# XinMing0411/AC-VAE

Measured on AMD Instinct MI355X. Metric: train-step captions/s (and audio-sec/s) at B=32, 1/2/4/8 MI355X, higher is better.
Workload: dtype f32

## Files before the change

acvae_amd/csrc/conv_wino.hip:

```cpp
#include "mfma_tile.h"
#include "../../include/acvae_hip.h"
#include "conv.h"
#include "prof.h"
#include <type_traits>

namespace {
using namespace mfma;

constexpr int WN_THREADS = 256;
constexpr int WN_TILES = 32;
constexpr int WN_TN = 64;
constexpr int WN_SC = 66, WN_SR = 2 * WN_SC, WN_SQ = 276;
constexpr int WN_BCHUNK = 16 * 2 * 64;
constexpr int WN_MAXC = 2048;
#ifndef WN_PRIO_EDGE
#define WN_PRIO_EDGE 3
#endif
#ifndef WN_PF_DIST
#define WN_PF_DIST 64
#endif

constexpr int WN_RAWBUF = 4 * WN_SQ;
constexpr int WN_EX_F4 = 6 * 512;
constexpr int WN_LDS_F4 = WN_EX_F4 + 64;
static_assert(2 * WN_RAWBUF <= WN_LDS_F4 && 2 * WN_RAWBUF + 2 * WN_MAXC / 4 >= WN_LDS_F4, "exchange + sums overlay the window buffers (+ scale / shift)");

__device__ __forceinline__ void wino_tile(int row, int tw_shift, int& tyl, int& tx) {
  const int cell = (int)((0x1c0c081804141000ULL >> (8 * (row >> 2))) & 0xff) + (row & 3);
  if (tw_shift >= 4) {
    tyl = cell >> tw_shift;
    tx = cell & ((1 << tw_shift) - 1);
  } else {
    const int g = cell >> 4, l16 = cell & 15;
    tx = l16 & ((1 << tw_shift) - 1);
    tyl = g + 2 * (l16 >> tw_shift);
  }
}
__host__ __device__ __forceinline__ int wino_row_pitch(int tw_shift) {
  return tw_shift == 3 ? 12 : tw_shift == 2 ? 6 : (1 << tw_shift) + 1;
}

struct WinoParams {
  const float* X;
  const float* scale;
  const float* shift;
  const float* U;
  float* Y;
  float* partials;
  const float* rY;
  const float* rscale;
  const float* rshift;
  const float* rmean;
  const float* rinvstd;
  int N, H, W, C, Cout;
  int tw_shift;
  int R;
  int bpc;
  int w_shift;
  unsigned bpc_magic;
  int nn_shift;
  int bn_group;
};
__device__ __forceinline__ void wino_tile_of(const WinoParams& p, int t, int nm, int nn, int& bm, int& bn) {
  if (p.bn_group) {
    const int G = p.bn_group, per = nm * G;
    int grp = (int)__fdividef((float)t, (float)per);
    int rem = t - grp * per;
    if (rem < 0) { --grp; rem += per; } else if (rem >= per) { ++grp; rem -= per; }
    bm = rem >> (G >> 1);
    bn = grp * G + (rem & (G - 1));
  } else if (p.nn_shift >= 0) { bn = t & (nn - 1); bm = t >> p.nn_shift; }
  else { bn = t % nn; bm = t / nn; }
}
__device__ __forceinline__ int wino_xcd_tile(const WinoParams& p, int nm, int nn, int& bm, int& bn) {
  const int total = nm * nn;
  const int b = blockIdx.x + blockIdx.y * nm;
  const int q = total >> 3, r = total & 7;
  const int xcd = b & 7, idx = b >> 3;
  const int t = xcd * q + (xcd < r ? xcd : r) + idx;
  wino_tile_of(p, t, nm, nn, bm, bn);
  return t;
}

typedef float f32x2 __attribute__((ext_vector_type(2)));
#define WN_PK_SUB(d, a, b) "v_pk_add_f32 " d ", " a ", " b " neg_lo:[0,1] neg_hi:[0,1]\n\t"
#define WN_PK_ADD(d, a, b) "v_pk_add_f32 " d ", " a ", " b "\n\t"
__device__ __forceinline__ float4 f4sub(float4 a, float4 b) {
  f32x2 lo, hi;
  asm(WN_PK_SUB("%0", "%2", "%4") WN_PK_SUB("%1", "%3", "%5")
      : "=&v"(lo), "=&v"(hi) : "v"(f32x2{a.x, a.y}), "v"(f32x2{a.z, a.w}), "v"(f32x2{b.x, b.y}), "v"(f32x2{b.z, b.w}));
  return make_float4(lo[0], lo[1], hi[0], hi[1]);
}
__device__ __forceinline__ float4 f4add(float4 a, float4 b) {
  f32x2 lo, hi;
  asm(WN_PK_ADD("%0", "%2", "%4") WN_PK_ADD("%1", "%3", "%5")
      : "=&v"(lo), "=&v"(hi) : "v"(f32x2{a.x, a.y}), "v"(f32x2{a.z, a.w}), "v"(f32x2{b.x, b.y}), "v"(f32x2{b.z, b.w}));
  return make_float4(lo[0], lo[1], hi[0], hi[1]);
}
__device__ __forceinline__ void wino_htrans(const float4 (&t)[4], float4 (&v)[4]) {
  f32x2 o[8];
  asm(WN_PK_SUB("%0", "%8", "%12") WN_PK_SUB("%1", "%9", "%13")
      WN_PK_ADD("%2", "%10", "%12") WN_PK_ADD("%3", "%11", "%13")
      WN_PK_SUB("%4", "%12", "%10") WN_PK_SUB("%5", "%13", "%11")
      WN_PK_SUB("%6", "%10", "%14") WN_PK_SUB("%7", "%11", "%15")
      "s_nop 1"
      : "=&v"(o[0]), "=&v"(o[1]), "=&v"(o[2]), "=&v"(o[3]), "=&v"(o[4]), "=&v"(o[5]), "=&v"(o[6]), "=&v"(o[7])
      : "v"(f32x2{t[0].x, t[0].y}), "v"(f32x2{t[0].z, t[0].w}), "v"(f32x2{t[1].x, t[1].y}), "v"(f32x2{t[1].z, t[1].w}),
        "v"(f32x2{t[2].x, t[2].y}), "v"(f32x2{t[2].z, t[2].w}), "v"(f32x2{t[3].x, t[3].y}), "v"(f32x2{t[3].z, t[3].w}));
#pragma unroll
  for (int k = 0; k < 4; ++k) v[k] = make_float4(o[2 * k][0], o[2 * k][1], o[2 * k + 1][0], o[2 * k + 1][1]);
}
__device__ __forceinline__ void pk_sub_ip(float4& a, const float4& b) {
  f32x2 lo{a.x, a.y}, hi{a.z, a.w};
  asm(WN_PK_SUB("%0", "%0", "%2") WN_PK_SUB("%1", "%1", "%3") : "+v"(lo), "+v"(hi) : "v"(f32x2{b.x, b.y}), "v"(f32x2{b.z, b.w}));
  a = make_float4(lo[0], lo[1], hi[0], hi[1]);
}
__device__ __forceinline__ void pk_add_ip(float4& a, const float4& b) {
  f32x2 lo{a.x, a.y}, hi{a.z, a.w};
  asm(WN_PK_ADD("%0", "%0", "%2") WN_PK_ADD("%1", "%1", "%3") : "+v"(lo), "+v"(hi) : "v"(f32x2{b.x, b.y}), "v"(f32x2{b.z, b.w}));
  a = make_float4(lo[0], lo[1], hi[0], hi[1]);
}
__device__ __forceinline__ void wino_htrans_ip(float4 (&t)[4], float4 (&v)[4]) {
  f32x2 a0{t[0].x, t[0].y}, a1{t[0].z, t[0].w}, c0{t[2].x, t[2].y}, c1{t[2].z, t[2].w}, e0{t[3].x, t[3].y}, e1{t[3].z, t[3].w};
  f32x2 n0, n1;
  asm(WN_PK_SUB("%0", "%0", "%2") WN_PK_SUB("%1", "%1", "%3")
      WN_PK_ADD("%6", "%8", "%2") WN_PK_ADD("%7", "%9", "%3")
      WN_PK_SUB("%2", "%2", "%8") WN_PK_SUB("%3", "%3", "%9")
      WN_PK_SUB("%4", "%8", "%4") WN_PK_SUB("%5", "%9", "%5")
      "s_nop 1"
      : "+v"(a0), "+v"(a1), "+v"(c0), "+v"(c1), "+v"(e0), "+v"(e1), "=&v"(n0), "=&v"(n1)
      : "v"(f32x2{t[1].x, t[1].y}), "v"(f32x2{t[1].z, t[1].w}));
  v[0] = make_float4(a0[0], a0[1], a1[0], a1[1]);
  v[1] = make_float4(n0[0], n0[1], n1[0], n1[1]);
  v[2] = make_float4(c0[0], c0[1], c1[0], c1[1]);
  v[3] = make_float4(e0[0], e0[1], e1[0], e1[1]);
}
__device__ __forceinline__ void mfma4_first(f32x16& c, float4 a, float4 b) {
  const f32x16 z = {0.f, 0.f, 0.f, 0.f, 0.f, 0.f, 0.f, 0.f, 0.f, 0.f, 0.f, 0.f, 0.f, 0.f, 0.f, 0.f};
  c = __builtin_amdgcn_mfma_f32_32x32x2f32(a.x, b.x, z, 0, 0, 0);
  c = __builtin_amdgcn_mfma_f32_32x32x2f32(a.y, b.y, c, 0, 0, 0);
  c = __builtin_amdgcn_mfma_f32_32x32x2f32(a.z, b.z, c, 0, 0, 0);
  c = __builtin_amdgcn_mfma_f32_32x32x2f32(a.w, b.w, c, 0, 0, 0);
}
__device__ __forceinline__ void mfma4(f32x16& c, float4 a, float4 b) {
  c = __builtin_amdgcn_mfma_f32_32x32x2f32(a.x, b.x, c, 0, 0, 0);
  c = __builtin_amdgcn_mfma_f32_32x32x2f32(a.y, b.y, c, 0, 0, 0);
  c = __builtin_amdgcn_mfma_f32_32x32x2f32(a.z, b.z, c, 0, 0, 0);
  c = __builtin_amdgcn_mfma_f32_32x32x2f32(a.w, b.w, c, 0, 0, 0);
}

template <int XI, int MODE>
__device__ __forceinline__ void wino_epilogue(const WinoParams& p, const f32x16 (&acc)[8], float2* ex, float* red, int li, int h,
                                              int lane, int n, int ty0, int bm, int bn) {
  constexpr int ROW = XI >> 1, NH = XI & 1;
  constexpr int SET_OTHER = XI == 0 ? 0 : XI == 1 ? 1 : XI == 2 ? 4 : 5;
  constexpr int SET_OWN = XI == 1 ? 2 : XI == 2 ? 3 : -1;
  constexpr int SET_A = XI == 0 ? 1 : XI == 1 ? 0 : XI == 2 ? 1 : 2, SET_B = XI == 0 ? 3 : XI == 1 ? 4 : XI == 2 ? 5 : 4;
  constexpr bool STATS = MODE != 0;
  const int tid = XI * 64 + lane;
  const int H = p.H, W = p.W, Cout = p.Cout;
  const int cout = bn * WN_TN + NH * 32 + li;
  int yk[4], voff[4];
#pragma unroll
  for (int k = 0; k < 4; ++k) {
    int tyl, tx;
    wino_tile(8 * k + 4 * h, p.tw_shift, tyl, tx);
    yk[k] = 2 * (ty0 + tyl) + ROW;
    voff[k] = ((yk[k] * W + 2 * tx) * Cout + cout) * 4;
  }
  int dyj[4], soff[4];
#pragma unroll
  for (int j = 0; j < 4; ++j) {
    dyj[j] = p.tw_shift == 1 ? 4 * (j >> 1) : 0;
    const int dx = p.tw_shift == 1 ? 2 * (j & 1) : 2 * j;
    soff[j] = (dyj[j] * W + dx) * Cout * 4;
  }
  const int pix = Cout * 4;
  float2 yv[MODE == 2 ? 16 : 1];
  float rsc = 0.f, rsh = 0.f, rmu = 0.f, ris = 0.f;
  if (MODE == 2) {
    const __amdgpu_buffer_rsrc_t rrs = __builtin_amdgcn_make_buffer_rsrc(const_cast<float*>(p.rY) + (long)n * H * W * Cout, 0, H * W * Cout * 4, 0x00020000);
#pragma unroll
    for (int r = 0; r < 16; ++r) {
      yv[r].x = __uint_as_float(__builtin_amdgcn_raw_buffer_load_b32(rrs, voff[r >> 2], soff[r & 3], 0));
      yv[r].y = __uint_as_float(__builtin_amdgcn_raw_buffer_load_b32(rrs, voff[r >> 2], soff[r & 3] + pix, 0));
    }
    rsc = p.rscale[cout]; rsh = p.rshift[cout]; rmu = p.rmean[cout]; ris = p.rinvstd[cout];
  }
  float2 keep[16];
#pragma unroll
  for (int r = 0; r < 16; ++r) {
#pragma unroll
    for (int nh = 0; nh < 2; ++nh) {
      const float m0 = acc[0 + nh][r], m1 = acc[2 + nh][r], m2 = acc[4 + nh][r], m3 = acc[6 + nh][r];
      const float2 f = make_float2(m0 + m1 + m2, m1 - m2 - m3);
      if (nh == NH) {
        keep[r] = f;
        if (SET_OWN >= 0) ex[(SET_OWN * 16 + r) * 64 + lane] = f;
      } else {
        ex[(SET_OTHER * 16 + r) * 64 + lane] = f;
      }
    }
  }
  __syncthreads();
  const __amdgpu_buffer_rsrc_t yrs = __builtin_amdgcn_make_buffer_rsrc(p.Y + (long)n * H * W * Cout, 0, H * W * Cout * 4, 0x00020000);
  float s = 0.f, qq = 0.f;
#pragma unroll
  for (int r = 0; r < 16; ++r) {
    const int k = r >> 2, j = r & 3;
    const float2 a = ex[(SET_A * 16 + r) * 64 + lane], b = ex[(SET_B * 16 + r) * 64 + lane];
    const float o0 = ROW ? a.x - (b.x + keep[r].x) : (keep[r].x + a.x) + b.x, o1 = ROW ? a.y - (b.y + keep[r].y) : (keep[r].y + a.y) + b.y;
    __builtin_amdgcn_raw_buffer_store_b32(__float_as_uint(o0), yrs, voff[k], soff[j], 0);
    __builtin_amdgcn_raw_buffer_store_b32(__float_as_uint(o1), yrs, voff[k], soff[j] + pix, 0);
    if (MODE == 1) {
      const bool ok = yk[k] + dyj[j] < H;
      const float a0 = ok ? o0 : 0.f, a1 = ok ? o1 : 0.f;
      s += a0 + a1;
      qq += a0 * a0 + a1 * a1;
    }
    if (MODE == 2) {
      const bool ok = yk[k] + dyj[j] < H;
      const float g0 = (ok && yv[r].x * rsc + rsh > 0.f) ? o0 : 0.f, g1 = (ok && yv[r].y * rsc + rsh > 0.f) ? o1 : 0.f;
      s += g0; s += g1;
      qq += g0 * ((yv[r].x - rmu) * ris); qq += g1 * ((yv[r].y - rmu) * ris);
    }
  }
  if (STATS && p.partials) {
    s += __shfl_xor(s, 32, 64);
    qq += __shfl_xor(qq, 32, 64);
    if (h == 0) {
      red[(ROW * 2 + 0) * 64 + NH * 32 + li] = s;
      red[(ROW * 2 + 1) * 64 + NH * 32 + li] = qq;
    }
    __syncthreads();
    if (tid < WN_TN) {
      const float ts = red[(0 * 2 + 0) * 64 + tid] + red[(1 * 2 + 0) * 64 + tid], tq = red[(0 * 2 + 1) * 64 + tid] + red[(1 * 2 + 1) * 64 + tid];
      float* out = p.partials + (long)bm * 2 * p.Cout + bn * WN_TN + tid;
      out[0] = ts;
      out[p.Cout] = tq;
    }
  }
}

template <int XI, bool ACT, int STATS>
__device__ __forceinline__ void conv_wino_body(const WinoParams& p, float4* raw0, float4* raw1, float4* scsh) {
  __builtin_amdgcn_s_setprio(WN_PRIO_EDGE);
  const int tid = threadIdx.x, lane = tid & 63;
  const int li = lane & 31, h = lane >> 5;
  int bm, bn;
  const int tpos = wino_xcd_tile(p, gridDim.x, gridDim.y, bm, bn);
  const int RW = wino_row_pitch(p.tw_shift), R = p.R;
  const int n = p.bpc == 1 ? bm : (int)__umulhi((unsigned)bm, p.bpc_magic), ty0 = (bm - n * p.bpc) * R;
  const int H = p.H, W = p.W, C = p.C;

  const int nitems = ((2 * R + 2) << p.w_shift) * 4;
  const int q = tid & 3;
  for (int i = tid; i < (2 * R + 2) * 8; i += WN_THREADS) {
    const int ry = i >> 3, side = (i >> 2) & 1, qi = i & 3;
    const int rx = side ? W + 1 : 0;
    const int slot = qi * WN_SQ + (ry & 1) * WN_SR + (rx & 1) * WN_SC + (ry >> 1) * RW + (rx >> 1);
    raw0[slot] = make_float4(0.f, 0.f, 0.f, 0.f);
    raw1[slot] = make_float4(0.f, 0.f, 0.f, 0.f);
  }
  unsigned goff[4];
  int loff[4];
#pragma unroll
  for (int j = 0; j < 4; ++j) {
    const int e = tid + WN_THREADS * j;
    const bool lv = e < nitems;
    const int px = e >> 2;
    const int ry = px >> p.w_shift, x = px & (W - 1), rx = x + 1;
    const int y = 2 * ty0 - 1 + ry;
    const bool ok = lv && y >= 0 && y < H;
    goff[j] = ok ? (unsigned)((((long)(n * H + y) * W + x) * C) + q * 4) : 0u;
    const int slot = q * WN_SQ + (ry & 1) * WN_SR + (rx & 1) * WN_SC + (ry >> 1) * RW + (rx >> 1);
    if (lv && !ok) {
      raw0[slot] = make_float4(0.f, 0.f, 0.f, 0.f);
      raw1[slot] = make_float4(0.f, 0.f, 0.f, 0.f);
    }
    loff[j] = ok ? slot : WN_RAWBUF - 1 - (tid & 7);
  }
  float4 pv[4];
  auto issue_raw = [&](int st) {
#pragma unroll
    for (int j = 0; j < 4; ++j) pv[j] = *reinterpret_cast<const float4*>(p.X + goff[j] + st * 16);
  };
  auto stage_scsh = [&]() {
    if (ACT) {
      for (int i = tid; i < (C >> 2); i += WN_THREADS) {
        scsh[i] = *reinterpret_cast<const float4*>(p.scale + 4 * i);
        scsh[(C >> 2) + i] = *reinterpret_cast<const float4*>(p.shift + 4 * i);
      }
      __syncthreads();
    }
  };
  float4 sc = make_float4(1.f, 1.f, 1.f, 1.f), sh = make_float4(0.f, 0.f, 0.f, 0.f);
  auto read_scsh = [&](int st) {
    if (ACT) {
      sc = scsh[st * 4 + q];
      sh = scsh[(C >> 2) + st * 4 + q];
    }
  };
  auto put_raw_part = [&](float4* raw, int j0) {
#pragma unroll
    for (int j = j0; j < j0 + 2; ++j) {
      float4 v = pv[j];
      if (ACT) {
        v.x = fmaxf(v.x * sc.x + sh.x, 0.f); v.y = fmaxf(v.y * sc.y + sh.y, 0.f);
        v.z = fmaxf(v.z * sc.z + sh.z, 0.f); v.w = fmaxf(v.w * sc.w + sh.w, 0.f);
      }
      raw[loff[j]] = v;
    }
  };
  auto put_raw = [&](float4* raw) { put_raw_part(raw, 0); put_raw_part(raw, 2); };
  const int nchunk = C >> 3;
  const __amdgpu_buffer_rsrc_t urs = __builtin_amdgcn_make_buffer_rsrc(
      const_cast<float*>(p.U + ((long)bn * nchunk) * (WN_BCHUNK * 4)), 0, 0x7fffffff, 0x00020000);
  int tyl_a, tx_a;
  wino_tile(li, p.tw_shift, tyl_a, tx_a);
  const int abase = tyl_a * RW + tx_a;
  constexpr int RA = XI == 0 ? 0 : XI == 2 ? 2 : 1, RB = XI == 0 ? 2 : XI == 1 ? 2 : XI == 2 ? 1 : 3;
  const int rowa = (RA & 1) * WN_SR + (RA >> 1) * RW + abase, rowb = (RB & 1) * WN_SR + (RB >> 1) * RW + abase;
  const int bvoff = (h * 64 + li) * 16;
  auto load_b = [&](int c, int g) {
    typedef unsigned wn_v4u __attribute__((ext_vector_type(4)));
    const wn_v4u v = __builtin_amdgcn_raw_buffer_load_b128(urs, bvoff, c * (WN_BCHUNK * 16) + (XI * 4 + (g >> 1)) * 2048 + (g & 1) * 512, 0);
    return make_float4(__uint_as_float(v.x), __uint_as_float(v.y), __uint_as_float(v.z), __uint_as_float(v.w));
  };

  f32x16 acc[8];

  const int nstage = C >> 4;
  const float4* const aq0 = raw0 + h * WN_SQ;
  const float4* const aq1 = raw1 + h * WN_SQ;
  float4 va[4], vb[4], B[4];
  auto read_row = [&](const float4* rq, int row, float4 (&d)[4]) {
#pragma unroll
    for (int j = 0; j < 4; ++j) d[j] = rq[row + (j & 1) * WN_SC + (j >> 1)];
  };
  auto vertical = [&](float4 (&da)[4], float4 (&db)[4]) {
#pragma unroll
    for (int j = 0; j < 4; ++j) {
      if (XI == 1) pk_add_ip(da[j], db[j]); else pk_sub_ip(da[j], db[j]);
    }
  };

#pragma unroll
  for (int g = 0; g < 4; ++g) B[g] = load_b(0, g);
  issue_raw(0);
  stage_scsh();
  read_scsh(0);
  put_raw(raw0);
  issue_raw(nstage > 1 ? 1 : 0);
  __syncthreads();
  {
    float4 da[4], db[4];
    read_row(aq0, rowa, da);
    read_row(aq0, rowb, db);
    vertical(da, db);
    wino_htrans_ip(da, va);
  }
#define WN_SB() __builtin_amdgcn_sched_barrier(0)
  auto step = [&](int c, auto kk, auto first) {
    constexpr int K = decltype(kk)::value;
    constexpr bool FIRST = decltype(first)::value;
    auto mm = [&](f32x16& a_, float4 x_, float4 y_) { if (FIRST) mfma4_first(a_, x_, y_); else mfma4(a_, x_, y_); };
    constexpr int sub = K & 1, sp = K >> 1;
    float4 (&vc)[4] = sub ? vb : va;
    float4 (&vn)[4] = sub ? va : vb;
    const int st = c >> 1;
    float4* const rnxt = sp ? raw0 : raw1;
    const float4* const nq = sub ? (sp ? aq0 : aq1) : (sp ? aq1 : aq0) + 2 * WN_SQ;
    const int cn = c + 1 < nchunk ? c + 1 : c;
    float4 da[4], db[4];
    const int st1 = st + 1 < nstage ? st + 1 : nstage - 1, st2 = st + 2 < nstage ? st + 2 : nstage - 1;
    if (sub == 0) read_scsh(st1);
    WN_SB();
    mm(acc[0], vc[0], B[0]);
    WN_SB();
    B[0] = load_b(c, 4);
    if (sub == 0) put_raw_part(rnxt, 0);
    WN_SB();
    mm(acc[1], vc[0], B[1]);
    WN_SB();
    B[1] = load_b(c, 5);
    if (sub == 0) put_raw_part(rnxt, 2);
    WN_SB();
    mm(acc[2], vc[1], B[2]);
    WN_SB();
    B[2] = load_b(c, 6);
    if (sub == 0) issue_raw(st2);
    WN_SB();
    mm(acc[3], vc[1], B[3]);
    WN_SB();
    B[3] = load_b(c, 7);
    read_row(nq, rowa, da);
    WN_SB();
    mm(acc[4], vc[2], B[0]);
    WN_SB();
    B[0] = load_b(cn, 0);
    read_row(nq, rowb, db);
    WN_SB();
    mm(acc[5], vc[2], B[1]);
    WN_SB();
    B[1] = load_b(cn, 1);
    WN_SB();
    mm(acc[6], vc[3], B[2]);
    WN_SB();
    B[2] = load_b(cn, 2);
    vertical(da, db);
    WN_SB();
    mm(acc[7], vc[3], B[3]);
    WN_SB();
    B[3] = load_b(cn, 3);
    wino_htrans_ip(da, vn);
    WN_SB();
    if (sub == 0) __syncthreads();
  };
#undef WN_SB
  using std::integral_constant;
  using std::false_type;
  __builtin_amdgcn_s_setprio(0);
  step(0, integral_constant<int, 0>(), std::true_type());
  step(1, integral_constant<int, 1>(), false_type());
  if (2 < nchunk) {
    step(2, integral_constant<int, 2>(), false_type());
    step(3, integral_constant<int, 3>(), false_type());
  }
  for (int c = 4; c < nchunk; c += 4) {
    step(c, integral_constant<int, 0>(), false_type());
    step(c + 1, integral_constant<int, 1>(), false_type());
    if (c + 2 < nchunk) {
      step(c + 2, integral_constant<int, 2>(), false_type());
      step(c + 3, integral_constant<int, 3>(), false_type());
    }
  }
  __builtin_amdgcn_s_setprio(WN_PRIO_EDGE);
  __syncthreads();
  const int lane_e = (int)__builtin_amdgcn_mbcnt_hi(~0u, __builtin_amdgcn_mbcnt_lo(~0u, 0u));
  const int li_e = lane_e & 31, h_e = lane_e >> 5;
  const int tid_e = XI * 64 + lane_e;

  float pfv = 0.f;
  if (!ACT) {
    const int nn_ = (int)gridDim.y;
    const int t2 = tpos + WN_PF_DIST * ((int)gridDim.x * nn_ >= 8 * WN_PF_DIST ? 1 : 0);
    int bm2 = bm, bn2 = bn;
    if (t2 < (int)gridDim.x * nn_) wino_tile_of(p, t2, (int)gridDim.x, nn_, bm2, bn2);
    const int n2 = p.bpc == 1 ? bm2 : (int)__umulhi((unsigned)bm2, p.bpc_magic), ty2 = (bm2 - n2 * p.bpc) * R;
    const int ry = tid_e >> p.w_shift, x = tid_e & (W - 1);
    const int y = 2 * ty2 - 1 + ry;
    if (bm2 < (int)gridDim.x && bm2 != bm && ry < 2 * R + 2 && y >= 0 && y < H)
      pfv = p.X[((long)(n2 * H + y) * W + x) * C];
  }

  float2* exb = reinterpret_cast<float2*>(raw0);
  wino_epilogue<XI, STATS>(p, acc, exb, reinterpret_cast<float*>(raw0 + WN_EX_F4),
                           li_e, h_e, lane_e, n, ty0, bm, bn);
  if (!ACT) asm volatile("" :: "v"(pfv));
}

template <bool ACT, int STATS>
__device__ __forceinline__ void conv_wino_entry(const WinoParams& p, float4* raw, float4* scsh) {
  switch (threadIdx.x >> 6) {
    case 0: conv_wino_body<0, ACT, STATS>(p, raw, raw + WN_RAWBUF, scsh); break;
    case 1: conv_wino_body<1, ACT, STATS>(p, raw, raw + WN_RAWBUF, scsh); break;
    case 2: conv_wino_body<2, ACT, STATS>(p, raw, raw + WN_RAWBUF, scsh); break;
    default: conv_wino_body<3, ACT, STATS>(p, raw, raw + WN_RAWBUF, scsh); break;
  }
}
__global__ __launch_bounds__(WN_THREADS, 2) void conv_wino_kernel(WinoParams p) {
  __shared__ float4 raw[WN_LDS_F4];
  conv_wino_entry<false, 0>(p, raw, nullptr);
}
__global__ __launch_bounds__(WN_THREADS, 2) void conv_wino_bnred_kernel(WinoParams p) {
  __shared__ float4 raw[WN_LDS_F4];
  conv_wino_entry<false, 2>(p, raw, nullptr);
}
__global__ __launch_bounds__(WN_THREADS, 2) void conv_wino_stats_kernel(WinoParams p) {
  __shared__ float4 raw[WN_LDS_F4];
  conv_wino_entry<false, 1>(p, raw, nullptr);
}
__global__ __launch_bounds__(WN_THREADS, 2) void conv_wino_act_kernel(WinoParams p) {
  __shared__ float4 raw[2 * WN_RAWBUF + 2 * WN_MAXC / 4];
  conv_wino_entry<true, 1>(p, raw, raw + 2 * WN_RAWBUF);
}

__device__ __forceinline__ void wino_weights_item(const float* __restrict__ Wt, float4* __restrict__ U, int Cout, int Cin, int dgrad,
                                                  long idx) {
  const int K = dgrad ? Cout : Cin, NO = dgrad ? Cin : Cout;
  {
    const int out = (int)(idx % NO), kq = (int)(idx / NO);
    float u[16][4];
#pragma unroll
    for (int jj = 0; jj < 4; ++jj) {
      const int in = kq * 4 + jj;
      double g[3][3];
#pragma unroll
      for (int a = 0; a < 3; ++a)
#pragma unroll
        for (int b = 0; b < 3; ++b)
          g[a][b] = dgrad ? (double)Wt[((long)in * Cin + out) * 9 + (2 - a) * 3 + (2 - b)]
                          : (double)Wt[((long)out * Cin + in) * 9 + a * 3 + b];
      double t[4][3];
#pragma unroll
      for (int b = 0; b < 3; ++b) {
        t[0][b] = g[0][b];
        t[1][b] = 0.5 * (g[0][b] + g[1][b] + g[2][b]);
        t[2][b] = 0.5 * (g[0][b] - g[1][b] + g[2][b]);
        t[3][b] = g[2][b];
      }
#pragma unroll
      for (int xi = 0; xi < 4; ++xi) {
        u[xi * 4 + 0][jj] = (float)t[xi][0];
        u[xi * 4 + 1][jj] = (float)(0.5 * (t[xi][0] + t[xi][1] + t[xi][2]));
        u[xi * 4 + 2][jj] = (float)(0.5 * (t[xi][0] - t[xi][1] + t[xi][2]));
        u[xi * 4 + 3][jj] = (float)t[xi][2];
      }
    }
    const int cb = out >> 6, col = out & 63, chunk = kq >> 1, hh = kq & 1;
    float4* dst = U + (((long)cb * (K >> 3) + chunk) * 16 * 2 + hh) * 64 + col;
#pragma unroll
    for (int pos = 0; pos < 16; ++pos) dst[(long)pos * 128] = make_float4(u[pos][0], u[pos][1], u[pos][2], u[pos][3]);
  }
}
__global__ void wino_weights_kernel(const float* __restrict__ Wt, float4* __restrict__ U, int Cout, int Cin, int dgrad) {
  const int K = dgrad ? Cout : Cin, NO = dgrad ? Cin : Cout;
  const long total = (long)NO * (K >> 2);
  for (long idx = blockIdx.x * (long)blockDim.x + threadIdx.x; idx < total; idx += (long)gridDim.x * blockDim.x)
    wino_weights_item(Wt, U, Cout, Cin, dgrad, idx);
}
__global__ void wino_weights_batch_kernel(acvae::WinoWeightsBatch b) {
  const long total = b.start[b.n];
  for (long idx = blockIdx.x * (long)blockDim.x + threadIdx.x; idx < total; idx += (long)gridDim.x * blockDim.x) {
    const int l = b.find(idx);
    const acvae::WinoWeightsJob& j = b.job[l];
    wino_weights_item(j.W, reinterpret_cast<float4*>(j.U), j.Cout, j.Cin, j.dgrad, idx - b.start[l]);
  }
}

inline int tile_rows_per_block(int W) { return WN_TILES / (W / 2); }
}

namespace acvae {

bool conv3x3_wino_ok(int H, int W, int Cin, int Cout) {
  if (H < 1 || W < 4 || W > 64 || (W & (W - 1)) != 0) return false;
  return Cin % 16 == 0 && Cin <= WN_MAXC && Cout % WN_TN == 0;
}
long conv3x3_wino_weight_floats(int Cin, int Cout) { return 16L * Cin * Cout; }
int conv_wino_partials_rows(int N, int H, int W) { return N * cdiv(cdiv(H, 2), tile_rows_per_block(W)); }

int conv3x3_wino_weights(const float* W_oihw, float* U, int Cout, int Cin, bool dgrad, hipStream_t st) {
  if (!W_oihw || !U) return ACVAE_EINVAL;
  const int K = dgrad ? Cout : Cin, NO = dgrad ? Cin : Cout;
  if (K % 16 != 0 || NO % WN_TN != 0) return ACVAE_EUNSUPPORTED;
  const long total = (long)NO * (K / 4);
  hipLaunchKernelGGL(wino_weights_kernel, dim3(cdiv(total, 256) > 4096 ? 4096 : cdiv(total, 256)), dim3(256), 0, st, W_oihw,
                     reinterpret_cast<float4*>(U), Cout, Cin, dgrad ? 1 : 0);
  ACVAE_LAUNCH_CHECK();
  return ACVAE_OK;
}

int conv3x3_wino_weights_batch(WinoWeightsBatch& b, hipStream_t st) {
  if (!b.ok()) return ACVAE_EINVAL;
  if (b.n <= 0) return ACVAE_OK;
  for (int l = 0; l < b.n; ++l) {
    const WinoWeightsJob& j = b.job[l];
    if (!j.W || !j.U) return ACVAE_EINVAL;
    const int K = j.dgrad ? j.Cout : j.Cin, NO = j.dgrad ? j.Cin : j.Cout;
    if (K % 16 != 0 || NO % WN_TN != 0) return ACVAE_EUNSUPPORTED;
  }
  const long total = b.seal([](const WinoWeightsJob& j) { return (long)j.Cout * j.Cin / 4; });
  hipLaunchKernelGGL(wino_weights_batch_kernel, dim3(cdiv(total, 256) > 8192 ? 8192 : cdiv(total, 256)), dim3(256), 0, st, b);
  ACVAE_LAUNCH_CHECK();
  return ACVAE_OK;
}

int conv3x3_wino(const float* X, const float* scale, const float* shift, const float* U, float* Y, float* partials, int N,
                 int H, int W, int Cin, int Cout, hipStream_t st, const WinoBnReduce* red) {
  if (!X || !U || !Y) return ACVAE_EINVAL;
  if (red && (scale || !partials || !red->Y || !red->scale || !red->shift || !red->mean || !red->invstd)) return ACVAE_EINVAL;
  if (!conv3x3_wino_ok(H, W, Cin, Cout)) return ACVAE_EUNSUPPORTED;
  if ((long)N * H * W * Cin >= (1L << 32)) return ACVAE_EUNSUPPORTED;
  if (!aligned16(X) || !aligned16(U) || !aligned16(Y) || (scale && (!aligned16(scale) || !aligned16(shift)))) return ACVAE_EALIGN;
  WinoParams p;
  p.X = X; p.scale = scale; p.shift = shift; p.U = U; p.Y = Y; p.partials = partials;
  p.rY = red ? red->Y : nullptr; p.rscale = red ? red->scale : nullptr; p.rshift = red ? red->shift : nullptr;
  p.rmean = red ? red->mean : nullptr; p.rinvstd = red ? red->invstd : nullptr;
  p.N = N; p.H = H; p.W = W; p.C = Cin; p.Cout = Cout;
  const int TW = W / 2;
  p.tw_shift = __builtin_ctz(TW);
  p.R = WN_TILES / TW;
  p.bpc = cdiv(cdiv(H, 2), p.R);
  p.w_shift = p.tw_shift + 1;
  p.bpc_magic = (unsigned)((0x100000000ULL + (unsigned)p.bpc - 1) / (unsigned)p.bpc);
  const int nn = Cout / WN_TN;
  p.nn_shift = (nn & (nn - 1)) == 0 ? __builtin_ctz(nn) : -1;
  {
    int G = 1;
    while (G < 4 && (long)(2 * G) * 4096 * Cin <= (2L << 20)) G *= 2;
    p.bn_group = (G < nn && nn % G == 0 && (long)nn * 4096 * Cin > (2L << 20) && (long)N * p.bpc * nn < (1L << 23)) ? G : 0;
  }
  if ((long)N * p.bpc >= (1L << 20)) return ACVAE_EUNSUPPORTED;
  const dim3 grid(N * p.bpc, Cout / WN_TN);
  prof_begin(ACVAE_PROF_CONV_IGEMM, st);
  if (red) hipLaunchKernelGGL(conv_wino_bnred_kernel, grid, dim3(WN_THREADS), 0, st, p);
  else if (scale) hipLaunchKernelGGL(conv_wino_act_kernel, grid, dim3(WN_THREADS), 0, st, p);
  else if (partials) hipLaunchKernelGGL(conv_wino_stats_kernel, grid, dim3(WN_THREADS), 0, st, p);
  else hipLaunchKernelGGL(conv_wino_kernel, grid, dim3(WN_THREADS), 0, st, p);
  prof_end(ACVAE_PROF_CONV_IGEMM, st);
  ACVAE_LAUNCH_CHECK();
  return ACVAE_OK;
}

}

namespace {
using namespace mfma;
constexpr int WG_XW_PIX = 136;
constexpr int WG_XW_WORDS = WG_XW_PIX * 64;
constexpr int WG_DY_WORDS = 16 * 4 * 64;

struct WinoWgradParams {
  const float* dY;
  const float* X;
  const float* scale;
  const float* shift;
  float* slab;
  int N, H, W, Cin, Cout;
  int st_shift;
  int RS;
  int segs;
  int spc;
  int total;
  int per;
};

template <int XI, int SS>
__device__ __forceinline__ void wino_wgrad_body(const WinoWgradParams& p, float* xw0, float* xw1, float* dy0, float* dy1) {
  const int tid = threadIdx.x, lane = tid & 63, wave = tid >> 6;
  const int li = lane & 31, kh = lane >> 5;
  const int wave_s = __builtin_amdgcn_readfirstlane(wave);
  const int ah = wave >> 2;
  const int z = blockIdx.x, cib = blockIdx.y, cob = blockIdx.z;
  const int H = p.H, W = p.W;
  constexpr int STW = 1 << SS, WC = 2 * STW + 2;
  const int WR = 2 * p.RS + 2;
  const int g_begin = z * p.per, g_end = min(p.total, g_begin + p.per);

  const int quad = tid & 15;
  int xyx[5], xlo[5];
  unsigned xlive = 0;
#pragma unroll
  for (int j = 0; j < 5; ++j) {
    const int e = tid + 512 * j, wp = e >> 4;
    const bool lv = wp < WR * WC;
    xlive |= (lv ? 1u : 0u) << j;
    const int wy = wp / WC, wx = wp - wy * WC;
    xyx[j] = (wy << 8) | wx;
    xlo[j] = wp * 64 + ((quad * 4) ^ (32 * ((wx >> 1) & 1)));
  }
  float4 sc = make_float4(1.f, 1.f, 1.f, 1.f), sh = make_float4(0.f, 0.f, 0.f, 0.f);
  const bool act = p.scale != nullptr;
  if (act) {
    sc = *reinterpret_cast<const float4*>(p.scale + cib * 64 + quad * 4);
    sh = *reinterpret_cast<const float4*>(p.shift + cib * 64 + quad * 4);
  }
  const int WCin = W * p.Cin;
  float4 px[5];
  unsigned xok = 0;
  const int seg_shift = p.segs == 2 ? 1 : 0;
  auto issue_dy = [&](int n, int s, float* dys) {
    const int trow = s >> seg_shift, seg = s & (p.segs - 1);
    const int ty0 = trow * p.RS, tx0 = seg * 16;
#pragma unroll
    for (int i = 0; i < 2; ++i) {
      const int t = wave * 2 + i, pp = lane >> 4, pq = lane & 15;
      const int y = 2 * (ty0 + (t >> p.st_shift)) + (pp >> 1), x = 2 * (tx0 + (t & (STW - 1))) + (pp & 1);
      float* dst = dys + t * 256;
      if (y < H) {
        const float* src = p.dY + (unsigned)(((n * H + y) * W + x) * p.Cout + cob * 64 + ((pq ^ (8 * (t & 1))) << 2));
        __builtin_amdgcn_global_load_lds(src, dst, 16, 0, 0);
      } else {
        *reinterpret_cast<float4*>(dst + lane * 4) = make_float4(0.f, 0.f, 0.f, 0.f);
      }
    }
  };
  auto issue_x = [&](int n, int s) {
    const int trow = s >> seg_shift, seg = s & (p.segs - 1);
    const int ty0 = trow * p.RS, tx0 = seg * 16;
    const int xbase = ((n * H + 2 * ty0 - 1) * W + (2 * tx0 - 1)) * p.Cin + cib * 64 + quad * 4;
    xok = 0;
#pragma unroll
    for (int j = 0; j < 5; ++j) {
      const int wy = xyx[j] >> 8, wx = xyx[j] & 255;
      const int y = 2 * ty0 - 1 + wy, x = 2 * tx0 - 1 + wx;
      const bool ok = ((xlive >> j) & 1u) && y >= 0 && y < H && x >= 0 && x < W;
      xok |= (ok ? 1u : 0u) << j;
      const unsigned off = ok ? (unsigned)(xbase + wy * WCin + wx * p.Cin) : 0u;
      px[j] = *reinterpret_cast<const float4*>(p.X + off);
    }
  };
  auto put_part = [&](float* xw, int j0, int j1) {
#pragma unroll
    for (int j = j0; j < j1; ++j) {
      float4 v = px[j];
      if (act) {
        v.x = fmaxf(v.x * sc.x + sh.x, 0.f); v.y = fmaxf(v.y * sc.y + sh.y, 0.f);
        v.z = fmaxf(v.z * sc.z + sh.z, 0.f); v.w = fmaxf(v.w * sc.w + sh.w, 0.f);
      }
      if (!((xok >> j) & 1u)) v = make_float4(0.f, 0.f, 0.f, 0.f);
      if ((xlive >> j) & 1u) *reinterpret_cast<float4*>(xw + xlo[j]) = v;
    }
  };

  const int ci = ah * 32 + li;
  const int xo01 = kh * 128 + (ci ^ (32 * kh)), xo23 = kh * 128 + (ci ^ (32 * (1 - kh)));
  constexpr int rowstride = WC * 64;
  const int bbase0 = kh * 256 + (li ^ (32 * kh)), bbase1 = kh * 256 + ((32 + li) ^ (32 * kh));
  constexpr int RA = XI == 0 ? 0 : 1, RB = XI == 0 ? 2 : XI == 3 ? 3 : 2;

  f32x16 acc[8];
#pragma unroll
  for (int i = 0; i < 8; ++i)
#pragma unroll
    for (int r = 0; r < 16; ++r) acc[i][r] = 0.f;

  struct Frag { float d[2][4]; float y[2][4]; };
  auto load = [&](auto jj, const float* xw, const float* dys, Frag& f) {
    constexpr int j = decltype(jj)::value;
    constexpr int OFF = ((2 * ((2 * j) >> SS)) * WC + 2 * ((2 * j) & (STW - 1))) * 64;
    const float* x01 = xw + xo01 + OFF;
    const float* x23 = xw + xo23 + OFF;
#pragma unroll
    for (int a = 0; a < 2; ++a) {
      constexpr int ROW[2] = {RA, RB};
      f.d[a][0] = x01[ROW[a] * rowstride + 0 * 64];
      f.d[a][1] = x01[ROW[a] * rowstride + 1 * 64];
      f.d[a][2] = x23[ROW[a] * rowstride + 2 * 64];
      f.d[a][3] = x23[ROW[a] * rowstride + 3 * 64];
    }
    const float* ya = dys + bbase0 + j * 512;
    const float* yb = dys + bbase1 + j * 512;
    f.y[0][0] = ya[0]; f.y[0][1] = ya[64]; f.y[0][2] = ya[128]; f.y[0][3] = ya[192];
    f.y[1][0] = yb[0]; f.y[1][1] = yb[64]; f.y[1][2] = yb[128]; f.y[1][3] = yb[192];
  };
#define WG_A01(D, TL, TH) "v_pk_add_f32 " D ", " TL ", " TH " op_sel_hi:[1,0] neg_lo:[0,1] neg_hi:[0,0]\n\t"
#define WG_A23(D, TL, TH) "v_pk_add_f32 " D ", " TH ", " TL " op_sel:[0,1] op_sel_hi:[1,1] neg_lo:[0,1] neg_hi:[0,1]\n\t"
#define WG_B12(D, R) "v_pk_add_f32 " D ", " R ", " R " op_sel:[0,1] op_sel_hi:[0,1] neg_lo:[0,0] neg_hi:[0,1]\n\t"
#define WG_SUB(D, A, B) "v_pk_add_f32 " D ", " A ", " B " neg_lo:[0,1] neg_hi:[0,1]\n\t"
#define WG_ADD(D, A, B) "v_pk_add_f32 " D ", " A ", " B "\n\t"
  auto mm = [&](const Frag& f) {
    f32x2 a01, a23, b12a, b12b, ra, rb;
    f32x2 tl = {f.d[0][0], f.d[0][1]}, th = {f.d[0][2], f.d[0][3]};
    const f32x2 ul = {f.d[1][0], f.d[1][1]}, uh = {f.d[1][2], f.d[1][3]};
    const f32x2 y0a = {f.y[0][0], f.y[0][1]}, y1a = {f.y[0][2], f.y[0][3]}, y0b = {f.y[1][0], f.y[1][1]}, y1b = {f.y[1][2], f.y[1][3]};
    if constexpr (XI == 0) {
      asm(WG_SUB("%4", "%4", "%6") WG_SUB("%5", "%5", "%7")
          WG_A01("%0", "%4", "%5") WG_A23("%1", "%4", "%5") WG_B12("%2", "%8") WG_B12("%3", "%9") "s_nop 1"
          : "=&v"(a01), "=&v"(a23), "=&v"(b12a), "=&v"(b12b), "+v"(tl), "+v"(th) : "v"(ul), "v"(uh), "v"(y0a), "v"(y0b));
      ra = y0a; rb = y0b;
    } else if constexpr (XI == 3) {
      asm(WG_SUB("%4", "%6", "%4") WG_SUB("%5", "%7", "%5")
          WG_A01("%0", "%4", "%5") WG_A23("%1", "%4", "%5") WG_B12("%2", "%8") WG_B12("%3", "%9") "s_nop 1"
          : "=&v"(a01), "=&v"(a23), "=&v"(b12a), "=&v"(b12b), "+v"(tl), "+v"(th) : "v"(ul), "v"(uh), "v"(y1a), "v"(y1b));
      ra = y1a; rb = y1b;
    } else if constexpr (XI == 1) {
      asm(WG_ADD("%6", "%6", "%8") WG_ADD("%7", "%7", "%9") WG_ADD("%4", "%10", "%11") WG_ADD("%5", "%12", "%13")
          WG_A01("%0", "%6", "%7") WG_A23("%1", "%6", "%7") WG_B12("%2", "%4") WG_B12("%3", "%5") "s_nop 1"
          : "=&v"(a01), "=&v"(a23), "=&v"(b12a), "=&v"(b12b), "=&v"(ra), "=&v"(rb), "+v"(tl), "+v"(th)
          : "v"(ul), "v"(uh), "v"(y0a), "v"(y1a), "v"(y0b), "v"(y1b));
    } else {
      asm(WG_SUB("%6", "%8", "%6") WG_SUB("%7", "%9", "%7") WG_SUB("%4", "%10", "%11") WG_SUB("%5", "%12", "%13")
          WG_A01("%0", "%6", "%7") WG_A23("%1", "%6", "%7") WG_B12("%2", "%4") WG_B12("%3", "%5") "s_nop 1"
          : "=&v"(a01), "=&v"(a23), "=&v"(b12a), "=&v"(b12b), "=&v"(ra), "=&v"(rb), "+v"(tl), "+v"(th)
          : "v"(ul), "v"(uh), "v"(y0a), "v"(y1a), "v"(y0b), "v"(y1b));
    }
    acc[0] = __builtin_amdgcn_mfma_f32_32x32x2f32(a01[0], ra[0], acc[0], 0, 0, 0);
    acc[1] = __builtin_amdgcn_mfma_f32_32x32x2f32(a01[0], rb[0], acc[1], 0, 0, 0);
    acc[2] = __builtin_amdgcn_mfma_f32_32x32x2f32(a01[1], b12a[0], acc[2], 0, 0, 0);
    acc[3] = __builtin_amdgcn_mfma_f32_32x32x2f32(a01[1], b12b[0], acc[3], 0, 0, 0);
    acc[4] = __builtin_amdgcn_mfma_f32_32x32x2f32(a23[0], b12a[1], acc[4], 0, 0, 0);
    acc[5] = __builtin_amdgcn_mfma_f32_32x32x2f32(a23[0], b12b[1], acc[5], 0, 0, 0);
    acc[6] = __builtin_amdgcn_mfma_f32_32x32x2f32(a23[1], ra[1], acc[6], 0, 0, 0);
    acc[7] = __builtin_amdgcn_mfma_f32_32x32x2f32(a23[1], rb[1], acc[7], 0, 0, 0);
  };
#undef WG_A01
#undef WG_A23
#undef WG_B12
#undef WG_SUB
#undef WG_ADD
#define WG_SB() __builtin_amdgcn_sched_barrier(0)
  auto compute = [&](const float* xw, const float* dys, bool more, int nn, int ns, float* xw_n, float* dy_n) {
    Frag fa, fb;
    load(std::integral_constant<int, 0>(), xw, dys, fa);
    load(std::integral_constant<int, 1>(), xw, dys, fb); WG_SB(); mm(fa); WG_SB();
    if (more) issue_dy(nn, ns, dy_n);
    WG_SB();
    load(std::integral_constant<int, 2>(), xw, dys, fa); WG_SB(); mm(fb); WG_SB();
    if (more) issue_x(nn, ns);
    WG_SB();
    load(std::integral_constant<int, 3>(), xw, dys, fb); WG_SB(); mm(fa); WG_SB();
    load(std::integral_constant<int, 4>(), xw, dys, fa); WG_SB(); mm(fb); WG_SB();
    load(std::integral_constant<int, 5>(), xw, dys, fb); WG_SB(); mm(fa); WG_SB();
    if (more) put_part(xw_n, 0, 2);
    WG_SB();
    load(std::integral_constant<int, 6>(), xw, dys, fa); WG_SB(); mm(fb); WG_SB();
    if (more) put_part(xw_n, 2, 4);
    WG_SB();
    load(std::integral_constant<int, 7>(), xw, dys, fb); WG_SB(); mm(fa); WG_SB();
    if (more) put_part(xw_n, 4, 5);
    WG_SB();
    mm(fb);
    WG_SB();
    asm volatile("s_waitcnt vmcnt(0)" ::: "memory");
    __syncthreads();
  };
#undef WG_SB

  if (g_begin < g_end) {
    int n = g_begin / p.spc, sidx = g_begin - n * p.spc;
    issue_dy(n, sidx, dy0);
    issue_x(n, sidx);
    put_part(xw0, 0, 5);
    asm volatile("s_waitcnt vmcnt(0)" ::: "memory");
    __syncthreads();
    for (int g = g_begin; g < g_end; g += 2) {
      if (++sidx == p.spc) { sidx = 0; ++n; }
      compute(xw0, dy0, g + 1 < g_end, n, sidx, xw1, dy1);
      if (g + 1 < g_end) {
        if (++sidx == p.spc) { sidx = 0; ++n; }
        compute(xw1, dy1, g + 2 < g_end, n, sidx, xw0, dy0);
      }
    }
  }

  const int lane_e = (int)__builtin_amdgcn_mbcnt_hi(~0u, __builtin_amdgcn_mbcnt_lo(~0u, 0u));
  const int li_e = lane_e & 31, kh_e = lane_e >> 5;
  const int ah_e = wave_s >> 2;
#pragma unroll
  for (int q = 0; q < 8; ++q) {
    const int pos = XI * 4 + (q >> 1);
    float* out = p.slab + (((long)z * 16 + pos) * p.Cin + cib * 64 + ah_e * 32) * p.Cout + cob * 64 + (q & 1) * 32 + li_e;
#pragma unroll
    for (int r = 0; r < 16; ++r) {
      const int row = (r & 3) + 8 * (r >> 2) + 4 * kh_e;
      out[(long)row * p.Cout] = acc[q][r];
    }
  }
}

template <int SS>
__device__ __forceinline__ void wino_wgrad_entry(const WinoWgradParams& p, float* xw0, float* xw1, float* dy0, float* dy1) {
  switch ((threadIdx.x >> 6) & 3) {
    case 0: wino_wgrad_body<0, SS>(p, xw0, xw1, dy0, dy1); break;
    case 1: wino_wgrad_body<1, SS>(p, xw0, xw1, dy0, dy1); break;
    case 2: wino_wgrad_body<2, SS>(p, xw0, xw1, dy0, dy1); break;
    default: wino_wgrad_body<3, SS>(p, xw0, xw1, dy0, dy1); break;
  }
}
#define WINO_WGRAD_KERNEL(SS)                                                                                    \
  __global__ __launch_bounds__(512) void conv_wino_wgrad_kernel_s##SS(WinoWgradParams p) {                     \
    __shared__ float xw0[WG_XW_WORDS], xw1[WG_XW_WORDS];                                                         \
    __shared__ float dy0[WG_DY_WORDS], dy1[WG_DY_WORDS];                                                         \
    wino_wgrad_entry<SS>(p, xw0, xw1, dy0, dy1);                                                                 \
  }
WINO_WGRAD_KERNEL(1) WINO_WGRAD_KERNEL(2) WINO_WGRAD_KERNEL(3) WINO_WGRAD_KERNEL(4)
#undef WINO_WGRAD_KERNEL

template <int PAIRS>
__global__ __launch_bounds__(256) void wino_wgrad_reduce_kernel(const float* __restrict__ slab, float* __restrict__ dW, int Z, int Cout,
                                                                int Cin) {
  constexpr int PG = 256 / PAIRS;
  constexpr int PPT = 16 / PG;
  __shared__ float su[16][PAIRS];
  const long total = (long)Cin * Cout, per_z = 16 * total;
  const int lp = threadIdx.x % PAIRS, pg = threadIdx.x / PAIRS;
  const long pair = (long)blockIdx.x * PAIRS + lp;
  if (pair < total) {
#pragma unroll
    for (int k = 0; k < PPT; ++k) {
      const int pos = pg * PPT + k;
      const long idx = (long)pos * total + pair;
      double s0 = 0.0, s1 = 0.0, s2 = 0.0, s3 = 0.0;
      int z = 0;
      for (; z + 4 <= Z; z += 4) {
        const float a = slab[(long)z * per_z + idx], b = slab[(long)(z + 1) * per_z + idx];
        const float c = slab[(long)(z + 2) * per_z + idx], d = slab[(long)(z + 3) * per_z + idx];
        s0 += (double)a; s1 += (double)b; s2 += (double)c; s3 += (double)d;
      }
      for (; z < Z; ++z) s0 += (double)slab[(long)z * per_z + idx];
      su[pos][lp] = (float)((s0 + s1) + (s2 + s3));
    }
  }
  __syncthreads();
  if (pg != 0 || pair >= total) return;
  const int co = (int)(pair % Cout), ci = (int)(pair / Cout);
  double u[16];
#pragma unroll
  for (int pos = 0; pos < 16; ++pos) u[pos] = (double)su[pos][lp];
  double t[3][4];
#pragma unroll
  for (int nu = 0; nu < 4; ++nu) {
    t[0][nu] = u[0 * 4 + nu] + 0.5 * (u[1 * 4 + nu] + u[2 * 4 + nu]);
    t[1][nu] = 0.5 * (u[1 * 4 + nu] - u[2 * 4 + nu]);
    t[2][nu] = 0.5 * (u[1 * 4 + nu] + u[2 * 4 + nu]) + u[3 * 4 + nu];
  }
  float* out = dW + ((long)co * Cin + ci) * 9;
#pragma unroll
  for (int a = 0; a < 3; ++a) {
    out[a * 3 + 0] = (float)(t[a][0] + 0.5 * (t[a][1] + t[a][2]));
    out[a * 3 + 1] = (float)(0.5 * (t[a][1] - t[a][2]));
    out[a * 3 + 2] = (float)(0.5 * (t[a][1] + t[a][2]) + t[a][3]);
  }
}

struct WgradPlan { int st_shift, RS, segs, spc, total, Z, per; };
inline WgradPlan wino_wgrad_plan(int N, int H, int W, int Cin, int Cout) {
  WgradPlan g;
  const int TW = W / 2, TH = (H + 1) / 2;
  const int STW = TW < 16 ? TW : 16;
  g.st_shift = __builtin_ctz(STW);
  g.RS = 16 / STW;
  g.segs = TW / STW;
  g.spc = TW >= 16 ? TH * g.segs : (TH + g.RS - 1) / g.RS;
  g.total = N * g.spc;
  const int blocks = (Cin / 64) * (Cout / 64);
  int Z = 256 / blocks;
  if (Z < 1) Z = 1;
  if (Z > g.total) Z = g.total;
  g.per = (g.total + Z - 1) / Z;
  g.Z = (g.total + g.per - 1) / g.per;
  return g;
}
}

namespace acvae {
bool conv3x3_wino_wgrad_ok(int H, int W, int Cin, int Cout) {
  if (H < 1 || W < 4 || W > 64 || (W & (W - 1)) != 0) return false;
  return Cin % 64 == 0 && Cout % 64 == 0;
}
static bool wino_wgrad_fits(int N, int H, int W, int Cin, int Cout) {
  return (long)N * H * W * (Cin > Cout ? Cin : Cout) < (1L << 31);
}
long conv3x3_wino_wgrad_slab_floats(int N, int H, int W, int Cin, int Cout) {
  if (!conv3x3_wino_wgrad_ok(H, W, Cin, Cout)) return 0;
  return (long)wino_wgrad_plan(N, H, W, Cin, Cout).Z * 16 * Cin * Cout;
}
int conv3x3_wino_wgrad(const float* dY, const float* X, const float* scale, const float* shift, float* dW_oihw, float* slab,
                       int N, int H, int W, int Cin, int Cout, hipStream_t st) {
  if (!dY || !X || !dW_oihw || !slab) return ACVAE_EINVAL;
  if (!conv3x3_wino_wgrad_ok(H, W, Cin, Cout) || !wino_wgrad_fits(N, H, W, Cin, Cout)) return ACVAE_EUNSUPPORTED;
  if (!aligned16(dY) || !aligned16(X) || !aligned16(slab) || (scale && (!aligned16(scale) || !aligned16(shift)))) return ACVAE_EALIGN;
  const WgradPlan g = wino_wgrad_plan(N, H, W, Cin, Cout);
  WinoWgradParams p;
  p.dY = dY; p.X = X; p.scale = scale; p.shift = shift; p.slab = slab;
  p.N = N; p.H = H; p.W = W; p.Cin = Cin; p.Cout = Cout;
  p.st_shift = g.st_shift; p.RS = g.RS; p.segs = g.segs; p.spc = g.spc; p.total = g.total; p.per = g.per;
  prof_begin(ACVAE_PROF_CONV_WGRAD, st);
  const dim3 wgrid(g.Z, Cin / 64, Cout / 64);
  switch (g.st_shift) {
    case 1: hipLaunchKernelGGL(conv_wino_wgrad_kernel_s1, wgrid, dim3(512), 0, st, p); break;
    case 2: hipLaunchKernelGGL(conv_wino_wgrad_kernel_s2, wgrid, dim3(512), 0, st, p); break;
    case 3: hipLaunchKernelGGL(conv_wino_wgrad_kernel_s3, wgrid, dim3(512), 0, st, p); break;
    default: hipLaunchKernelGGL(conv_wino_wgrad_kernel_s4, wgrid, dim3(512), 0, st, p); break;
  }
  prof_end(ACVAE_PROF_CONV_WGRAD, st);
  const long total = (long)Cin * Cout;
  if (total < 16 * 1024)
    hipLaunchKernelGGL(wino_wgrad_reduce_kernel<16>, dim3((unsigned)cdiv(total, 16)), dim3(256), 0, st, slab, dW_oihw, g.Z, Cout, Cin);
  else
    hipLaunchKernelGGL(wino_wgrad_reduce_kernel<64>, dim3((unsigned)cdiv(total, 64)), dim3(256), 0, st, slab, dW_oihw, g.Z, Cout, Cin);
  ACVAE_LAUNCH_CHECK();
  return ACVAE_OK;
}
}
```

Measured before the change: 2117.

## Streamline Winograd wgrad loads with buffer loads, precomputed offsets and static pad zeroing

Reworks the input/dY staging of the Winograd weight-gradient kernel. X loads now go through raw buffer loads with hardware out-of-bounds clipping and precomputed per-thread offsets, so the per-element bounds checks go away. The always-zero padding columns are written once per LDS buffer, and padded slots are redirected to a dummy LDS area. dY loads use precomputed offsets with a fast path for interior rows. The activation path is specialized at compile time and uses packed FMA plus med3 clamping. The prefetch at the tail is made unconditional, which adds redundant loads at the end, and a new size limit narrows which shapes can use the kernel.

```diff
diff --git a/acvae_amd/csrc/conv_wino.hip b/acvae_amd/csrc/conv_wino.hip
--- a/acvae_amd/csrc/conv_wino.hip
+++ b/acvae_amd/csrc/conv_wino.hip
@@ -619,7 +619,7 @@
 namespace {
 using namespace mfma;
 constexpr int WG_XW_PIX = 136;
-constexpr int WG_XW_WORDS = WG_XW_PIX * 64;
+constexpr int WG_XW_WORDS = WG_XW_PIX * 64 + 64;
 constexpr int WG_DY_WORDS = 16 * 4 * 64;
 
 struct WinoWgradParams {
@@ -646,20 +646,31 @@
   const int z = blockIdx.x, cib = blockIdx.y, cob = blockIdx.z;
   const int H = p.H, W = p.W;
   constexpr int STW = 1 << SS, WC = 2 * STW + 2;
-  const int WR = 2 * p.RS + 2;
+  constexpr int RS = 16 >> SS, WR = 2 * RS + 2;
   const int g_begin = z * p.per, g_end = min(p.total, g_begin + p.per);
 
   const int quad = tid & 15;
-  int xyx[5], xlo[5];
-  unsigned xlive = 0;
+  const bool two = SS == 4 && p.segs == 2;
+  const int seg_b0 = two ? (g_begin & 1) : 0;
+  unsigned xoff[5];
+  int xlo0[5], xlo1[5];
 #pragma unroll
   for (int j = 0; j < 5; ++j) {
     const int e = tid + 512 * j, wp = e >> 4;
     const bool lv = wp < WR * WC;
-    xlive |= (lv ? 1u : 0u) << j;
     const int wy = wp / WC, wx = wp - wy * WC;
-    xyx[j] = (wy << 8) | wx;
-    xlo[j] = wp * 64 + ((quad * 4) ^ (32 * ((wx >> 1) & 1)));
+    const bool padl = wx == 0, padr = wx == WC - 1;
+    const bool pad0 = two ? (seg_b0 ? padr : padl) : (padl || padr), pad1 = two ? (seg_b0 ? padl : padr) : (padl || padr);
+    const int slot = wp * 64 + ((quad * 4) ^ (32 * ((wx >> 1) & 1))), dummy = WG_XW_PIX * 64 + quad * 4;
+    xoff[j] = lv ? (unsigned)(((wy * W + wx) * p.Cin + quad * 4) * 4) : 0x80000000u;
+    xlo0[j] = lv && !pad0 ? slot : dummy;
+    xlo1[j] = lv && !pad1 ? slot : dummy;
+  }
+  for (int i = tid; i < WR * 32; i += 512) {
+    const int wy = i >> 5, side = (i >> 4) & 1, wx = side ? WC - 1 : 0;
+    const int slot = (wy * WC + wx) * 64 + (i & 15) * 4;
+    if (!two || side == seg_b0) *reinterpret_cast<float4*>(xw0 + slot) = make_float4(0.f, 0.f, 0.f, 0.f);
+    if (!two || side != seg_b0) *reinterpret_cast<float4*>(xw1 + slot) = make_float4(0.f, 0.f, 0.f, 0.f);
   }
   float4 sc = make_float4(1.f, 1.f, 1.f, 1.f), sh = make_float4(0.f, 0.f, 0.f, 0.f);
   const bool act = p.scale != nullptr;
@@ -667,51 +678,66 @@
     sc = *reinterpret_cast<const float4*>(p.scale + cib * 64 + quad * 4);
     sh = *reinterpret_cast<const float4*>(p.shift + cib * 64 + quad * 4);
   }
-  const int WCin = W * p.Cin;
+  unsigned dyoff[2];
+#pragma unroll
+  for (int i = 0; i < 2; ++i) {
+    const int t = wave * 2 + i, pp = lane >> 4, pq = lane & 15;
+    dyoff[i] = (unsigned)(((2 * (t >> SS) + (pp >> 1)) * W + 2 * (t & (STW - 1)) + (pp & 1)) * p.Cout + ((pq ^ (8 * i)) << 2));
+  }
+  const unsigned clip_bytes = (unsigned)(H * W * p.Cin) * 4u;
   float4 px[5];
-  unsigned xok = 0;
+  bool xin[5];
   const int seg_shift = p.segs == 2 ? 1 : 0;
   auto issue_dy = [&](int n, int s, float* dys) {
     const int trow = s >> seg_shift, seg = s & (p.segs - 1);
-    const int ty0 = trow * p.RS, tx0 = seg * 16;
-#pragma unroll
-    for (int i = 0; i < 2; ++i) {
-      const int t = wave * 2 + i, pp = lane >> 4, pq = lane & 15;
-      const int y = 2 * (ty0 + (t >> p.st_shift)) + (pp >> 1), x = 2 * (tx0 + (t & (STW - 1))) + (pp & 1);
-      float* dst = dys + t * 256;
-      if (y < H) {
-        const float* src = p.dY + (unsigned)(((n * H + y) * W + x) * p.Cout + cob * 64 + ((pq ^ (8 * (t & 1))) << 2));
-        __builtin_amdgcn_global_load_lds(src, dst, 16, 0, 0);
-      } else {
-        *reinterpret_cast<float4*>(dst + lane * 4) = make_float4(0.f, 0.f, 0.f, 0.f);
+    const int ty0 = trow * RS, tx0 = seg * 16;
+    const float* sbase = p.dY + (unsigned)(((n * H + 2 * ty0) * W + 2 * tx0) * p.Cout + cob * 64);
+    if (2 * (ty0 + RS) <= H) {
+#pragma unroll
+      for (int i = 0; i < 2; ++i) __builtin_amdgcn_global_load_lds(sbase + dyoff[i], dys + (wave_s * 2 + i) * 256, 16, 0, 0);
+    } else {
+      const int lane_d = (int)__builtin_amdgcn_mbcnt_hi(~0u, __builtin_amdgcn_mbcnt_lo(~0u, 0u));
+#pragma unroll
+      for (int i = 0; i < 2; ++i) {
+        const int t = wave_s * 2 + i;
+        float* dst = dys + t * 256;
+        if (2 * (ty0 + (t >> SS)) + (lane_d >> 5) < H) __builtin_amdgcn_global_load_lds(sbase + dyoff[i], dst, 16, 0, 0);
+        else *reinterpret_cast<float4*>(dst + lane_d * 4) = make_float4(0.f, 0.f, 0.f, 0.f);
       }
     }
   };
-  auto issue_x = [&](int n, int s) {
+  auto issue_x = [&](auto actt, int n, int s) {
+    constexpr bool ACT = decltype(actt)::value;
     const int trow = s >> seg_shift, seg = s & (p.segs - 1);
-    const int ty0 = trow * p.RS, tx0 = seg * 16;
-    const int xbase = ((n * H + 2 * ty0 - 1) * W + (2 * tx0 - 1)) * p.Cin + cib * 64 + quad * 4;
-    xok = 0;
+    const int ty0 = trow * RS, tx0 = seg * 16;
+    const unsigned xbase = (unsigned)((((2 * ty0 - 1) * W + (2 * tx0 - 1)) * p.Cin + cib * 64) * 4);
+    const __amdgpu_buffer_rsrc_t xrs =
+        __builtin_amdgcn_make_buffer_rsrc(const_cast<float*>(p.X) + (unsigned)(n * H * W * p.Cin), 0, (int)clip_bytes, 0x00020000);
 #pragma unroll
     for (int j = 0; j < 5; ++j) {
-      const int wy = xyx[j] >> 8, wx = xyx[j] & 255;
-      const int y = 2 * ty0 - 1 + wy, x = 2 * tx0 - 1 + wx;
-      const bool ok = ((xlive >> j) & 1u) && y >= 0 && y < H && x >= 0 && x < W;
-      xok |= (ok ? 1u : 0u) << j;
-      const unsigned off = ok ? (unsigned)(xbase + wy * WCin + wx * p.Cin) : 0u;
-      px[j] = *reinterpret_cast<const float4*>(p.X + off);
-    }
-  };
-  auto put_part = [&](float* xw, int j0, int j1) {
+      typedef unsigned wg_v4u __attribute__((ext_vector_type(4)));
+      const unsigned off = xoff[j] + xbase;
+      const wg_v4u v = __builtin_amdgcn_raw_buffer_load_b128(xrs, (int)off, 0, 0);
+      px[j] = make_float4(__uint_as_float(v.x), __uint_as_float(v.y), __uint_as_float(v.z), __uint_as_float(v.w));
+      if (ACT) xin[j] = off < clip_bytes;
+    }
+  };
+  auto put_part = [&](auto actt, float* xw, const int (&xlo)[5], int j0, int j1) {
+    constexpr bool ACT = decltype(actt)::value;
 #pragma unroll
     for (int j = j0; j < j1; ++j) {
       float4 v = px[j];
-      if (act) {
-        v.x = fmaxf(v.x * sc.x + sh.x, 0.f); v.y = fmaxf(v.y * sc.y + sh.y, 0.f);
-        v.z = fmaxf(v.z * sc.z + sh.z, 0.f); v.w = fmaxf(v.w * sc.w + sh.w, 0.f);
+      if (ACT) {
+        const float lim = xin[j] ? __builtin_inff() : 0.f;
+        f32x2 lo, hi;
+        asm("v_pk_mul_f32 %0, %2, %4\n\tv_pk_mul_f32 %1, %3, %5\n\tv_pk_add_f32 %0, %0, %6\n\tv_pk_add_f32 %1, %1, %7"
+            : "=&v"(lo), "=&v"(hi)
+            : "v"(f32x2{v.x, v.y}), "v"(f32x2{v.z, v.w}), "v"(f32x2{sc.x, sc.y}), "v"(f32x2{sc.z, sc.w}), "v"(f32x2{sh.x, sh.y}),
+              "v"(f32x2{sh.z, sh.w}));
+        v.x = __builtin_amdgcn_fmed3f(lo[0], 0.f, lim); v.y = __builtin_amdgcn_fmed3f(lo[1], 0.f, lim);
+        v.z = __builtin_amdgcn_fmed3f(hi[0], 0.f, lim); v.w = __builtin_amdgcn_fmed3f(hi[1], 0.f, lim);
       }
-      if (!((xok >> j) & 1u)) v = make_float4(0.f, 0.f, 0.f, 0.f);
-      if ((xlive >> j) & 1u) *reinterpret_cast<float4*>(xw + xlo[j]) = v;
+      *reinterpret_cast<float4*>(xw + xlo[j]) = v;
     }
   };
 
@@ -792,25 +818,25 @@
 #undef WG_SUB
 #undef WG_ADD
 #define WG_SB() __builtin_amdgcn_sched_barrier(0)
-  auto compute = [&](const float* xw, const float* dys, bool more, int nn, int ns, float* xw_n, float* dy_n) {
+  auto compute = [&](auto actt, const float* xw, const float* dys, int nn, int ns, float* xw_n, const int (&xlo_n)[5], float* dy_n) {
     Frag fa, fb;
     load(std::integral_constant<int, 0>(), xw, dys, fa);
     load(std::integral_constant<int, 1>(), xw, dys, fb); WG_SB(); mm(fa); WG_SB();
-    if (more) issue_dy(nn, ns, dy_n);
+    issue_dy(nn, ns, dy_n);
     WG_SB();
     load(std::integral_constant<int, 2>(), xw, dys, fa); WG_SB(); mm(fb); WG_SB();
-    if (more) issue_x(nn, ns);
+    issue_x(actt, nn, ns);
     WG_SB();
     load(std::integral_constant<int, 3>(), xw, dys, fb); WG_SB(); mm(fa); WG_SB();
     load(std::integral_constant<int, 4>(), xw, dys, fa); WG_SB(); mm(fb); WG_SB();
     load(std::integral_constant<int, 5>(), xw, dys, fb); WG_SB(); mm(fa); WG_SB();
-    if (more) put_part(xw_n, 0, 2);
+    put_part(actt, xw_n, xlo_n, 0, 2);
     WG_SB();
     load(std::integral_constant<int, 6>(), xw, dys, fa); WG_SB(); mm(fb); WG_SB();
-    if (more) put_part(xw_n, 2, 4);
+    put_part(actt, xw_n, xlo_n, 2, 4);
     WG_SB();
     load(std::integral_constant<int, 7>(), xw, dys, fb); WG_SB(); mm(fa); WG_SB();
-    if (more) put_part(xw_n, 4, 5);
+    put_part(actt, xw_n, xlo_n, 4, 5);
     WG_SB();
     mm(fb);
     WG_SB();
@@ -819,21 +845,24 @@
   };
 #undef WG_SB
 
-  if (g_begin < g_end) {
+  auto run = [&](auto actt) {
     int n = g_begin / p.spc, sidx = g_begin - n * p.spc;
     issue_dy(n, sidx, dy0);
-    issue_x(n, sidx);
-    put_part(xw0, 0, 5);
+    issue_x(actt, n, sidx);
+    put_part(actt, xw0, xlo0, 0, 5);
     asm volatile("s_waitcnt vmcnt(0)" ::: "memory");
     __syncthreads();
     for (int g = g_begin; g < g_end; g += 2) {
-      if (++sidx == p.spc) { sidx = 0; ++n; }
-      compute(xw0, dy0, g + 1 < g_end, n, sidx, xw1, dy1);
+      if (g + 1 < g_end && ++sidx == p.spc) { sidx = 0; ++n; }
+      compute(actt, xw0, dy0, n, sidx, xw1, xlo1, dy1);
       if (g + 1 < g_end) {
-        if (++sidx == p.spc) { sidx = 0; ++n; }
-        compute(xw1, dy1, g + 2 < g_end, n, sidx, xw0, dy0);
+        if (g + 2 < g_end && ++sidx == p.spc) { sidx = 0; ++n; }
+        compute(actt, xw1, dy1, n, sidx, xw0, xlo0, dy0);
       }
     }
+  };
+  if (g_begin < g_end) {
+    if (act) run(std::true_type()); else run(std::false_type());
   }
 
   const int lane_e = (int)__builtin_amdgcn_mbcnt_hi(~0u, __builtin_amdgcn_mbcnt_lo(~0u, 0u));
@@ -942,7 +971,7 @@
   return Cin % 64 == 0 && Cout % 64 == 0;
 }
 static bool wino_wgrad_fits(int N, int H, int W, int Cin, int Cout) {
-  return (long)N * H * W * (Cin > Cout ? Cin : Cout) < (1L << 31);
+  return (long)N * H * W * (Cin > Cout ? Cin : Cout) < (1L << 31) && (long)H * W * Cin * 4 <= (1L << 30);
 }
 long conv3x3_wino_wgrad_slab_floats(int N, int H, int W, int Cin, int Cout) {
   if (!conv3x3_wino_wgrad_ok(H, W, Cin, Cout)) return 0;
```

Result: faster. 2160 (median of 6 runs) (+2.0%).
